# RyanXLi/OneshotDet

Hardware: AMD Instinct MI355X
Metric: images/sec/GPU fwd+bwd, 800x1024 target + 127x127 query, bs=8; 1->8 GPU scaling (higher is better)
Workload: dtype bf16; 1 GPU; BASELINE.json configs[2]: bs=8/GPU, 800x1024 target + 127x127 query, bf16 MFMA convs, forward (two R-50-FPN backbones, query pooling, correlation, FCOS head, training proposals) + FCOS loss + backward (stem/layer1 frozen) + gradient all-reduce + SGD(momentum) + weight repack; global_batch=8, parallelism=dp1: one rank, no collective anywhere in the step, world_size=1

## Files before the change

oneshotdet_amd/csrc/conv_wgrad.hip:

```cpp
#include "wgrad_params.h"

namespace {

__device__ __attribute__((aligned(256))) unsigned g_wzero[64];

__device__ __forceinline__ void wg_dma16(const void* gsrc, unsigned lds_dst) {
  unsigned keep;
  asm volatile(
      "s_mov_b32 %0, m0\n\ts_mov_b32 m0, %2\n\ts_nop 0\n\tglobal_load_lds_dwordx4 %1, off\n\ts_mov_b32 m0, %0"
      : "=&s"(keep)
      : "v"(gsrc), "s"(lds_dst)
      : "memory");
}

template <typename T, int BKP, int NST, int WCO, int WCI, int WM, int WN, bool ILV = false>
__global__ void __launch_bounds__(64 * WM * WN, (WM * WN == 4 && WCO + WCI == 3) ? 2 : 1) conv_wgrad_kernel(WgradParams gp) {
  constexpr int NW = WM * WN;
  constexpr int EPC = 16 / (int)sizeof(T);
  constexpr int TWS = 256 / (int)sizeof(T);
  constexpr int TCO = WCO * TWS, TCI = WCI * TWS;
  constexpr int OPB = BKP * 256;
  constexpr int STAGE = (WCO + WCI) * OPB;
  constexpr int PPS = BKP / 4;
  constexpr int IPA = WCO * PPS / NW;
// ... 747 lines not shown
__global__ void pred_wgrad_reduce_kernel(const float* __restrict__ part, const float* __restrict__ part_b, float* __restrict__ dw,
                                         float* __restrict__ db, int blocks, int groups, int C, int cout) {
  const int i = blockIdx.x * blockDim.x + threadIdx.x;
  const int n = cout * 9 * C;
  const int per = (blocks + gridDim.y - 1) / gridDim.y;
  const int b0 = blockIdx.y * per, b1 = min(blocks, b0 + per);
  if (i < n) {
    const int c = i % C, ct = i / C;
    const int cg = c >> 8, cl = c & 255;
    const size_t stride = (size_t)groups * 36 * 256;
    const float* p = part + ((size_t)cg * 36 + ct) * 256 + cl;
    float s0 = 0.f, s1 = 0.f, s2 = 0.f, s3 = 0.f;
    int b = b0;
    for (; b + 3 < b1; b += 4) {
      s0 += p[(size_t)b * stride]; s1 += p[(size_t)(b + 1) * stride]; s2 += p[(size_t)(b + 2) * stride]; s3 += p[(size_t)(b + 3) * stride];
    }
    for (; b < b1; ++b) s0 += p[(size_t)b * stride];
    if (b0 < b1) atomicAdd(dw + i, (s0 + s1) + (s2 + s3));
  } else if (db != nullptr && i < n + cout) {
    const int co = i - n;
    float s = 0.f;
    for (int b = b0 * 4; b < b1 * 4; ++b) s += part_b[(size_t)b * 4 + co];
    if (b0 < b1) atomicAdd(db + co, s);
  }
}

template <typename T>
__global__ void __launch_bounds__(256) bias_grad_kernel(const T* __restrict__ dy, float* __restrict__ db, int M, int C,
                                                        int stride, int rows_per_block) {
  const int c = blockIdx.y * blockDim.x + threadIdx.x;
  const int p_lo = blockIdx.x * rows_per_block, p_hi = min(M, p_lo + rows_per_block);
  if (c >= C || p_lo >= p_hi) return;
  float s = 0.f;
  for (int m = p_lo; m < p_hi; ++m) s += to_f32(dy[(size_t)m * stride + c]);
  atomicAdd(db + c, s);
}

}

#define OSD_STREAM(s) reinterpret_cast<hipStream_t>(s)

extern "C" int osd_bias_grad(const void* dy, float* db, int m, int c, int stride, int dtype, void* stream);

static bool wgrad_dense_input(const osd_conv_desc* d) {
  return d->in_stride_w == d->cin && d->in_stride_h == d->w * d->cin && (long long)d->in_stride_n == (long long)d->h * d->w * d->cin;
}

struct WgradProblem {
  const osd_conv_desc* d;
  int n, h, w;
  const void* x; const void* dy; const float* scale; float* dw; float* db;
};

static int wgrad_xr_launch(int n_seg, const WgradProblem* pr, hipStream_t s) {
  if (n_seg < 1 || n_seg > kMaxSeg) return osd_fail(OSD_ERR_INVALID_ARG, "wgrad: 1..%d segments", kMaxSeg);
  const osd_conv_desc* d0 = pr[0].d;
  static const int kTargets[8] = {512, 256, 128, 64, 1024, 768, 1536, 2048};
  const int a = d0->algo - 1 - 128;
  const int x = a & 15, target = kTargets[(a >> 4) & 7];
  if (a < 0 || a >= 128 || x > 2) return osd_fail(OSD_ERR_INVALID_ARG, "wgrad: unknown algo %d", d0->algo);
  const int bkp = x == 1 ? 64 : 32;
  WgradParams p;
  p.n_seg = n_seg;
  p.sk_units = 0;
  long long work = 0;
  for (int i = 0; i < n_seg; ++i) {
    const osd_conv_desc* d = pr[i].d;
    WgradSeg& g = p.seg[i];
    g.owner = 0;
    const int h = pr[i].h, w = pr[i].w;
    if (d->dtype != OSD_BF16 || d->r != 3 || d->s != 3 || d->stride_h != 1 || d->stride_w != 1 || d->pad_h != 1 || d->pad_w != 1 ||
        d->cout % 128 || d->cin % 128 || d->out_stride % 8 || !(w % bkp == 0 || bkp % w == 0))
      return osd_fail(OSD_ERR_UNSUPPORTED, "wgrad (filter-row kernel): bf16 3x3 / 1 / 1, channels in 128s, width %d vs %d-pixel stages", w, bkp);
    const long long M = (long long)pr[i].n * h * w;
    if (M <= 0 || M > 0x7fffffffLL || !pr[i].x || !pr[i].dy || !pr[i].dw) return osd_fail(OSD_ERR_INVALID_ARG, "wgrad: bad segment %d", i);
    if (M * d->cin > 0x7fffffffLL) return osd_fail(OSD_ERR_UNSUPPORTED, "wgrad: input of segment %d has more than 2^31 elements", i);
    g.x = pr[i].x; g.dy = pr[i].dy; g.dw = pr[i].dw; g.scale = pr[i].scale; g.db = pr[i].db;
    g.H = h; g.W = w; g.Ho = h; g.Wo = w; g.M = (int)M;
    g.Cin = d->cin; g.Cout = d->cout; g.R = 3; g.S = 3; g.sh = g.sw = 1; g.ph = g.pw = 1;
    g.dy_stride = d->out_stride; g.Ktot = 9 * d->cin;
    g.tilesCo = d->cout / 128; g.tilesCi = d->cin / 128;
    work += M * g.tilesCo * g.tilesCi * 3;
  }
  long long rows = (work + target - 1) / target;
  rows = (rows + 63) / 64 * 64;
  if (rows < 128) rows = 128;
  long long nblocks = 0;
  for (int i = 0; i < n_seg; ++i) {
    WgradSeg& g = p.seg[i];
    int sp = (int)((g.M + rows - 1) / rows);
    if (sp < 1) sp = 1;
    g.rows_per_split = cdiv(cdiv(g.M, sp), 64) * 64;
    const int splits = cdiv(g.M, g.rows_per_split);
    g.block_begin = (int)nblocks;
    nblocks += (long long)g.tilesCo * g.tilesCi * 3 * splits;
    if (nblocks > 0x7fffffffLL) return osd_fail(OSD_ERR_INVALID_ARG, "wgrad: bad grid");
  }
  for (int i = n_seg; i < kMaxSeg; ++i) p.seg[i] = p.seg[0];
  p.n_blocks = (int)nblocks;
  p.partials = nullptr;
#define OSD_WGX(BK, NS)                                                                                               \
  do {                                                                                                                \
    auto kern = conv_wgrad_xr_kernel<BK, NS>;                                                                         \
    constexpr int lds = NS * (BK + BK + 4) * 256;                                                                     \
    static bool attr = false;                                                                                         \
    if (!attr) { (void)hipFuncSetAttribute(reinterpret_cast<const void*>(kern), hipFuncAttributeMaxDynamicSharedMemorySize, lds); attr = true; } \
    hipLaunchKernelGGL(kern, dim3((unsigned)nblocks), dim3(512), lds, s, p);                                         \
  } while (0)
  if (x == 0) OSD_WGX(32, 6);
  else if (x == 1) OSD_WGX(64, 4);
  else OSD_WGX(32, 8);
#undef OSD_WGX
  return osd_check_launch("conv_wgrad_xr");
}

static int wgrad_launch_v(int n_seg, const WgradProblem* pr, hipStream_t s, int variant_override);
static int wgrad_launch(int n_seg, const WgradProblem* pr, hipStream_t s) {
  int rc = wgrad_launch_v(n_seg, pr, s, -1);
  if (rc == OSD_ERR_UNSUPPORTED && n_seg >= 1 && pr[0].d->algo == 0) rc = wgrad_launch_v(n_seg, pr, s, 0);
  return rc;
}

static int wgrad_launch_v(int n_seg, const WgradProblem* pr, hipStream_t s, int variant_override) {
  if (n_seg < 1 || n_seg > kMaxSeg) return osd_fail(OSD_ERR_INVALID_ARG, "wgrad: 1..%d segments", kMaxSeg);
  const osd_conv_desc* d0 = pr[0].d;
  if (d0->algo > 128) return wgrad_xr_launch(n_seg, pr, s);
  static int env_target = -1, env_variant = -1;
  if (env_target < 0) { const char* e = getenv("OSD_WGRAD_BLOCKS"); env_target = e ? atoi(e) : 512; }
  if (env_variant < 0) { const char* e = getenv("OSD_WGRAD_VARIANT"); env_variant = e ? atoi(e) : 0; }
  static const int kTargets[8] = {512, 256, 128, 64, 1024, 768, 1536, 2048};
  int target = env_target, variant = variant_override >= 0 ? variant_override : env_variant, code = 0;
  if (d0->algo > 0) {
    const int a = d0->algo - 1;
    if (a >= 128) return osd_fail(OSD_ERR_INVALID_ARG, "wgrad: unknown algo %d", d0->algo);
    variant = a & 15;
    code = a >> 4;
    target = kTargets[code];
  }
  if (d0->dtype == OSD_F32) target *= 8;
  const bool bf = d0->dtype == OSD_BF16;
  if (!bf && variant != 0) variant = 0;
  const int sub_co = bf && (variant == 3 || variant == 4 || variant == 5 || variant == 7 || variant == 8 || variant == 9 || variant == 11 || variant == 13 || variant == 14) ? 2 : 1;
  const int sub_ci = bf && (variant == 3 || variant == 4 || variant == 5 || variant == 6 || variant == 8 || variant == 9 || variant == 10 || variant == 13) ? 2 : 1;
  const int tw = bf ? 128 : 64;
  const int epc = d0->dtype == OSD_BF16 ? 8 : 4;
  WgradParams p;
  p.n_seg = n_seg;
  long long work = 0;
  for (int i = 0; i < n_seg; ++i) {
    const osd_conv_desc* d = pr[i].d;
    WgradSeg& g = p.seg[i];
    if (d->dtype != d0->dtype) return osd_fail(OSD_ERR_INVALID_ARG, "wgrad: segments of different dtype");
    if (d->cin % epc || d->out_stride % epc) return osd_fail(OSD_ERR_INVALID_ARG, "wgrad: channel counts must keep 16-byte alignment");
    const int ho = (pr[i].h + 2 * d->pad_h - d->r) / d->stride_h + 1, wo = (pr[i].w + 2 * d->pad_w - d->s) / d->stride_w + 1;
    const long long M = (long long)pr[i].n * ho * wo;
    if (M <= 0 || M > 0x7fffffffLL || !pr[i].x || !pr[i].dy || !pr[i].dw) return osd_fail(OSD_ERR_INVALID_ARG, "wgrad: bad segment %d", i);
    if ((long long)pr[i].n * pr[i].h * pr[i].w * d->cin > 0x7fffffffLL)
      return osd_fail(OSD_ERR_UNSUPPORTED, "wgrad: input of segment %d has more than 2^31 elements", i);
    g.x = pr[i].x; g.dy = pr[i].dy; g.dw = pr[i].dw; g.scale = pr[i].scale; g.db = pr[i].db;
    g.H = pr[i].h; g.W = pr[i].w; g.Ho = ho; g.Wo = wo; g.M = (int)M;
    g.Cin = d->cin; g.Cout = d->cout; g.R = d->r; g.S = d->s;
    g.sh = d->stride_h; g.sw = d->stride_w; g.ph = d->pad_h; g.pw = d->pad_w;
    g.dy_stride = d->out_stride; g.Ktot = d->r * d->s * d->cin;
    g.tilesCo = cdiv(d->cout, tw * sub_co); g.tilesCi = cdiv(d->cin, tw * sub_ci);
    work += M * g.tilesCo * g.tilesCi * d->r * d->s;
  }
  long long rows = (work + target - 1) / target;
  rows = (rows + 31) / 32 * 32;
  if (rows < 128) rows = 128;
  long long nblocks = 0;
  for (int i = 0; i < n_seg; ++i) {
    WgradSeg& g = p.seg[i];
    int sp = (int)((g.M + rows - 1) / rows);
    if (sp < 1) sp = 1;
    g.rows_per_split = cdiv(cdiv(g.M, sp), 32) * 32;
    const int splits = cdiv(g.M, g.rows_per_split);
    g.owner = splits == 1 ? 1 : 0;
    g.block_begin = (int)nblocks;
    nblocks += (long long)g.tilesCo * g.tilesCi * g.R * g.S * splits;
    if (nblocks > 0x7fffffffLL) return osd_fail(OSD_ERR_INVALID_ARG, "wgrad: bad grid");
  }
  p.sk_units = p.sk_teams = p.sk_total = 0;
  if (bf && variant == 3) {
    if (d0->ordered_ws != nullptr) return osd_fail(OSD_ERR_UNSUPPORTED, "wgrad: team mode adds its partial tiles atomically (not for ordered mode)");
    if (code > 3) return osd_fail(OSD_ERR_UNSUPPORTED, "wgrad: team mode knows target codes 0..3 (rounds)");
    const WgradSeg& g0 = p.seg[0];
    long long total = 0;
    for (int i = 0; i < n_seg; ++i) {
      WgradSeg& g = p.seg[i];
      if (g.Cout != g0.Cout || g.Cin != g0.Cin || g.R != g0.R || g.S != g0.S)
        return osd_fail(OSD_ERR_UNSUPPORTED, "wgrad: team mode needs segments of one conv shape (segment %d differs)", i);
      g.stage_begin = (int)total;
      total += cdiv(g.M, 64);
    }
    static int cus = 0;
    if (cus == 0) {
      int dev = 0;
      if (hipGetDevice(&dev) != hipSuccess || hipDeviceGetAttribute(&cus, hipDeviceAttributeMultiprocessorCount, dev) != hipSuccess || cus < 1) cus = 256;
      const char* e = getenv("OSD_WGRAD_TEAM_CUS");
      if (e && atoi(e) > 0) cus = atoi(e);
    }
    const int units = g0.tilesCo * g0.tilesCi * g0.R * g0.S;
    long long teams = (long long)cus * (code + 1) / units;
    if (teams < 1) return osd_fail(OSD_ERR_UNSUPPORTED, "wgrad: team mode needs at most one output tile x tap per CU (%d)", units);
    if (teams > total) teams = total;
    if (total > 0x7fffffffLL) return osd_fail(OSD_ERR_INVALID_ARG, "wgrad: bad grid");
    p.sk_units = units; p.sk_teams = (int)teams; p.sk_total = (int)total;
    nblocks = teams * units;
  }
  static int no_owner = -1;
  if (no_owner < 0) { const char* e = getenv("OSD_WGRAD_NO_OWNER"); no_owner = (e && atoi(e) != 0) ? 1 : 0; }
  for (int i = 0; i < n_seg; ++i) {
    if (no_owner || d0->ordered_ws != nullptr || p.sk_units > 0) p.seg[i].owner = 0;
    for (int j = 0; j < n_seg && p.seg[i].owner; ++j)
      if (j != i && p.seg[j].dw == p.seg[i].dw) p.seg[i].owner = 0;
  }
  for (int i = n_seg; i < kMaxSeg; ++i) p.seg[i] = p.seg[0];
  p.n_blocks = (int)nblocks;
  p.partials = nullptr;
  const int tco = tw * sub_co, tci = tw * sub_ci;
  if (d0->ordered_ws != nullptr) {
    const long long need = nblocks * ((long long)tco * tci + tco) * 4;
    if (need > (long long)d0->ordered_ws_bytes)
      return osd_fail(OSD_ERR_WORKSPACE, "wgrad (ordered mode): the launch needs %lld bytes of partial tiles, ordered_ws_bytes is %lld",
                      need, (long long)d0->ordered_ws_bytes);
    p.partials = static_cast<float*>(d0->ordered_ws);
  }
  const osd_conv_desc* d = d0;
#define OSD_WG_LAUNCH(TT, BK, NS, WC, WMM, WNN) OSD_WG_LAUNCH3(TT, BK, NS, WC, WC, WMM, WNN, false)
#define OSD_WG_LAUNCH2(TT, BK, NS, WCOO, WCII, WMM, WNN) OSD_WG_LAUNCH3(TT, BK, NS, WCOO, WCII, WMM, WNN, false)
#define OSD_WG_LAUNCH3(TT, BK, NS, WCOO, WCII, WMM, WNN, IL)                                                        \
  do {                                                                                                               \
    auto kern = conv_wgrad_kernel<TT, BK, NS, WCOO, WCII, WMM, WNN, IL>;                                                 \
    constexpr int lds = NS * (WCOO + WCII) * BK * 256;                                                               \
    static bool attr = false;                                                                                        \
    if (!attr) { (void)hipFuncSetAttribute(reinterpret_cast<const void*>(kern), hipFuncAttributeMaxDynamicSharedMemorySize, lds); attr = true; } \
    hipLaunchKernelGGL(kern, dim3((unsigned)nblocks), dim3(64 * WMM * WNN), lds, s, p);                             \
  } while (0)
  if (d->dtype == OSD_F32) {
    OSD_WG_LAUNCH(float, 32, 3, 1, 2, 2);
  } else {
    switch (variant) {
      case 1: OSD_WG_LAUNCH(__bf16, 64, 2, 1, 2, 2); break;
      case 2: OSD_WG_LAUNCH(__bf16, 32, 4, 1, 2, 2); break;
      case 4: OSD_WG_LAUNCH(__bf16, 32, 3, 2, 2, 4); break;
      case 5: OSD_WG_LAUNCH(__bf16, 64, 2, 2, 2, 4); break;
      case 6: OSD_WG_LAUNCH2(__bf16, 64, 2, 1, 2, 2, 4); break;
      case 7: OSD_WG_LAUNCH2(__bf16, 64, 2, 2, 1, 4, 2); break;
      case 8: OSD_WG_LAUNCH(__bf16, 32, 5, 2, 2, 4); break;
      case 9: OSD_WG_LAUNCH(__bf16, 32, 4, 2, 2, 4); break;
      case 10: OSD_WG_LAUNCH2(__bf16, 32, 3, 1, 2, 2, 2); break;
      case 11: OSD_WG_LAUNCH2(__bf16, 32, 3, 2, 1, 2, 2); break;
      case 12: return osd_fail(OSD_ERR_UNSUPPORTED, "wgrad: variant 12 is retired");
      case 3:
      case 13: {
        for (int i = 0; i < n_seg; ++i) {
          const WgradSeg& g = p.seg[i];
          if (g.Wo < 2 || g.Ho < 2 || (long long)g.M * g.Wo >= 0xffffffffLL || (long long)g.M * g.dy_stride * 2 >= 0x7fffffffLL ||
              (long long)(g.M / (g.Ho * g.Wo)) * g.H * g.W * g.Cin * 2 >= 0x7fffffffLL)
            return osd_fail(OSD_ERR_UNSUPPORTED, "wgrad: the pipelined variants need output maps of at least 2 x 2 and operands below 2 GiB (segment %d)", i);
        }
        const int rc = osd_wgrad_sk_launch(p, s);
        if (rc) return rc;
        break;
      }
      case 14: OSD_WG_LAUNCH3(__bf16, 32, 3, 2, 1, 2, 2, true); break;
      case 15: OSD_WG_LAUNCH3(__bf16, 32, 3, 1, 1, 2, 2, true); break;
      default: OSD_WG_LAUNCH(__bf16, 32, 3, 1, 2, 2); break;
    }
  }
#undef OSD_WG_LAUNCH
#undef OSD_WG_LAUNCH2
#undef OSD_WG_LAUNCH3
  if (p.partials != nullptr) {
    int rc = osd_check_launch("conv_wgrad");
    if (rc) return rc;
    long long tiles = 0;
    for (int i = 0; i < n_seg; ++i) tiles += (long long)p.seg[i].tilesCo * p.seg[i].tilesCi * p.seg[i].R * p.seg[i].S;
    hipLaunchKernelGGL(wgrad_reduce_kernel, dim3((unsigned)tiles, tco / 16), dim3(256), 0, s, p, tco, tci);
    return osd_check_launch("conv_wgrad(reduce)");
  }
  return osd_check_launch("conv_wgrad");
}

extern "C" int osd_conv2d_wgrad(const osd_conv_desc* d, const void* x, const void* dy, const float* scale, float* dw,
                                float* db, void* stream) {
  if (!d || !x || !dy || !dw) return osd_fail(OSD_ERR_INVALID_ARG, "wgrad: null argument");
  if (d->dtype != OSD_F32 && d->dtype != OSD_BF16) return osd_fail(OSD_ERR_INVALID_ARG, "wgrad: bad dtype");
  const int epc = d->dtype == OSD_BF16 ? 8 : 4;
  const long long M = (long long)d->n * d->ho * d->wo;
  if (M <= 0 || M > 0x7fffffffLL) return osd_fail(OSD_ERR_INVALID_ARG, "wgrad: bad M");
  if (!wgrad_dense_input(d)) return osd_fail(OSD_ERR_UNSUPPORTED, "wgrad: dense NHWC input required");
  hipStream_t s = OSD_STREAM(stream);
  if (d->cout <= 8 && (d->out_stride % epc != 0 || d->cin % epc != 0)) {
    if (d->r * d->s > 9) return osd_fail(OSD_ERR_UNSUPPORTED, "wgrad: skinny kernel supports up to 9 taps");
    const int rows = 512;
    dim3 grid(cdiv((int)M, rows), cdiv(d->cin, 256));
    if (d->dtype == OSD_F32)
      hipLaunchKernelGGL(conv_wgrad_skinny_kernel<float>, grid, dim3(256), 0, s, (const float*)x, (const float*)dy, dw, d->h,
                         d->w, d->cin, d->ho, d->wo, d->cout, d->r, d->s, d->stride_h, d->pad_h, d->out_stride, (int)M, rows);
    else
      hipLaunchKernelGGL(conv_wgrad_skinny_kernel<__bf16>, grid, dim3(256), 0, s, (const __bf16*)x, (const __bf16*)dy, dw,
                         d->h, d->w, d->cin, d->ho, d->wo, d->cout, d->r, d->s, d->stride_h, d->pad_h, d->out_stride, (int)M,
                         rows);
    int rc = osd_check_launch("conv_wgrad_skinny");
    if (rc || !db) return rc;
    return osd_bias_grad(dy, db, (int)M, d->cout, d->out_stride, d->dtype, stream);
  }
  const WgradProblem pr = {d, d->n, d->h, d->w, x, dy, scale, dw, db};
  return wgrad_launch(1, &pr, s);
}

extern "C" int osd_conv2d_wgrad_grouped(const osd_conv_desc* d, int n_seg, const void* const* xs, const void* const* dys,
                                        const int32_t* ns, const int32_t* hs, const int32_t* ws, const float* scale,
// ... 216 lines not shown
  const unsigned blocks = (unsigned)cdiv(cin * kPredG, 256);
  if (dtype == OSD_F32)
    hipLaunchKernelGGL(pred_dgrad_pack_kernel<float>, dim3(blocks), dim3(256), 0, OSD_STREAM(stream), w, (float*)wd, cout, cin);
  else
    hipLaunchKernelGGL(pred_dgrad_pack_kernel<__bf16>, dim3(blocks), dim3(256), 0, OSD_STREAM(stream), w, (__bf16*)wd, cout, cin);
  return osd_check_launch("pred_dgrad_pack");
}

extern "C" int osd_conv2d_wgrad_pred_gathered(const osd_conv_desc* d, int n_seg, const void* const* xs, const void* g, const int32_t* ns,
                                              const int32_t* hs, const int32_t* ws, float* dw, float* db, void* workspace, void* stream) {
  if (!xs || !g || !dw || !workspace) return osd_fail(OSD_ERR_INVALID_ARG, "wgrad_pred_gathered: null argument");
  int rc = pred_check("wgrad_pred_gathered", d, n_seg, ns, hs, ws);
  if (rc) return rc;
  for (int i = 0; i < n_seg; ++i)
    if (!xs[i]) return osd_fail(OSD_ERR_INVALID_ARG, "wgrad_pred_gathered: null segment %d", i);
  return pred_wgrad_from_g(d, n_seg, xs, g, ns, hs, ws, dw, db, workspace, OSD_STREAM(stream));
}

extern "C" int osd_conv2d_wgrad_batched(const osd_conv_desc* d, int n_seg, const void* const* xs, const void* const* dys,
                                        const float* const* scales, float* const* dws, float* const* dbs, void* stream) {
  if (!d || !xs || !dys || !dws || n_seg < 1 || n_seg > kMaxSeg)
    return osd_fail(OSD_ERR_INVALID_ARG, "wgrad_batched: bad arguments");
  if (d->dtype != OSD_F32 && d->dtype != OSD_BF16) return osd_fail(OSD_ERR_INVALID_ARG, "wgrad: bad dtype");
  if (!wgrad_dense_input(d)) return osd_fail(OSD_ERR_UNSUPPORTED, "wgrad_batched: dense NHWC input required");
  WgradProblem pr[kMaxSeg];
  for (int i = 0; i < n_seg; ++i)
    pr[i] = WgradProblem{d, d->n, d->h, d->w, xs[i], dys[i], scales ? scales[i] : nullptr, dws[i], dbs ? dbs[i] : nullptr};
  return wgrad_launch(n_seg, pr, OSD_STREAM(stream));
}

extern "C" int osd_conv2d_wgrad_multi(const osd_conv_desc* d, int n_seg, const void* const* xs, const void* const* dys,
                                      const int32_t* ns, const int32_t* hs, const int32_t* ws, const float* const* scales,
                                      float* const* dws, float* const* dbs, void* stream) {
  if (!d || !xs || !dys || !ns || !hs || !ws || !dws || n_seg < 1 || n_seg > kMaxSeg)
    return osd_fail(OSD_ERR_INVALID_ARG, "wgrad_multi: bad arguments (1..%d segments)", kMaxSeg);
  if (d->dtype != OSD_F32 && d->dtype != OSD_BF16) return osd_fail(OSD_ERR_INVALID_ARG, "wgrad: bad dtype");
  WgradProblem pr[kMaxSeg];
  for (int i = 0; i < n_seg; ++i)
    pr[i] = WgradProblem{d, ns[i], hs[i], ws[i], xs[i], dys[i], scales ? scales[i] : nullptr, dws[i], dbs ? dbs[i] : nullptr};
  return wgrad_launch(n_seg, pr, OSD_STREAM(stream));
}

extern "C" int osd_conv2d_wgrad_mixed(int n_seg, const osd_conv_desc* descs, const void* const* xs, const void* const* dys,
                                      const float* const* scales, float* const* dws, float* const* dbs, void* stream) {
  if (!descs || !xs || !dys || !dws || n_seg < 1 || n_seg > kMaxSeg)
    return osd_fail(OSD_ERR_INVALID_ARG, "wgrad_mixed: bad arguments (1..%d segments)", kMaxSeg);
  if (descs[0].dtype != OSD_F32 && descs[0].dtype != OSD_BF16) return osd_fail(OSD_ERR_INVALID_ARG, "wgrad: bad dtype");
  WgradProblem pr[kMaxSeg];
  for (int i = 0; i < n_seg; ++i) {
    const osd_conv_desc* d = descs + i;
    if (!wgrad_dense_input(d)) return osd_fail(OSD_ERR_UNSUPPORTED, "wgrad_mixed: dense NHWC input required (segment %d)", i);
    pr[i] = WgradProblem{d, d->n, d->h, d->w, xs[i], dys[i], scales ? scales[i] : nullptr, dws[i], dbs ? dbs[i] : nullptr};
  }
  return wgrad_launch(n_seg, pr, OSD_STREAM(stream));
}

extern "C" int osd_bias_grad(const void* dy, float* db, int m, int c, int stride, int dtype, void* stream) {
  if (!dy || !db) return osd_fail(OSD_ERR_INVALID_ARG, "bias_grad: null argument");
  if (m == 0 || c == 0) return OSD_OK;
  const int rows = m > 65536 ? 2048 : 512;
  dim3 grid(cdiv(m, rows), cdiv(c, 256));
  if (dtype == OSD_F32)
    hipLaunchKernelGGL(bias_grad_kernel<float>, grid, dim3(256), 0, OSD_STREAM(stream), (const float*)dy, db, m, c, stride, rows);
  else if (dtype == OSD_BF16)
    hipLaunchKernelGGL(bias_grad_kernel<__bf16>, grid, dim3(256), 0, OSD_STREAM(stream), (const __bf16*)dy, db, m, c, stride,
                       rows);
  else
    return osd_fail(OSD_ERR_INVALID_ARG, "bias_grad: bad dtype");
  return osd_check_launch("bias_grad");
}
```

oneshotdet_amd/ops.py:

```python
import ctypes as C
import os

import torch

from . import _lib, spec
from ._lib import (ACT_EXP_SCALE, ACT_NONE, ACT_RELU, GN_SPLITS, OSD_BF16, OSD_F32, RES_DOWN2X, RES_NONE, RES_SAME, RES_UP2X,
                   ConvDesc)

__all__ = ["ACT_NONE", "ACT_RELU", "ACT_EXP_SCALE", "RES_NONE", "RES_SAME", "RES_UP2X", "RES_DOWN2X"]


from . import streams

_stream_handle = streams.raw_handle


def _stream():
    return C.c_void_p(_stream_handle())


from .trace import rec as _rec
from . import trace as _trace


# ... 51 lines not shown
        scale = (g * var.rsqrt()).contiguous()
        fbias = b - mean * scale
    else:
        fbias = bias.float() if bias is not None else torch.zeros(cout, device=weight.device)
    cout_store = _round_up(cout, 4)
    w_rows = _round_up(cout, 16)
    bias_p = torch.zeros(_round_up(cout_store, 16), device=weight.device, dtype=torch.float32)
    bias_p[:cout] = fbias
    if stem:
        assert (cin, r, s) == (3, 7, 7)
        wp = torch.empty((w_rows, 7, 32), device=weight.device, dtype=dtype)
        _lib.call("osd_pack_stem_weight", _p(weight), _p(scale), _p(wp), cout, w_rows, _dt(wp), _stream())
        return PackedConv(wp, bias_p, cout, cout_store, w_rows, 32, 7, 1, stem=True, cin_real=3)
    mult = 64 if dtype == torch.bfloat16 else 16
    cin_pad = _round_up(cin, mult)
    wp = torch.empty((w_rows, r, s, cin_pad), device=weight.device, dtype=dtype)
    _lib.call("osd_pack_conv_weight", _p(weight), _p(scale), _p(wp), cout, cin, r, s, w_rows, cin_pad, _dt(wp),
              _stream())
    return PackedConv(wp, bias_p, cout, cout_store, w_rows, cin_pad, r, s, cin_real=cin)


def pack_image(images, dtype, hp, wp, pad_t=3, pad_l=3):
    _chk_dev(images)
    n, c, h, w = images.shape
    assert c == 3 and images.dtype == torch.float32
    out = torch.empty((n, hp, wp, 4), device=images.device, dtype=dtype)
    _lib.call("osd_pack_image", _ptr(images.contiguous()), _p(out), n, h, w, hp, wp, pad_t, pad_l, _dt(out), _stream())
    _rec("pack_image", x=images, out=out, pad_t=pad_t, pad_l=pad_l)
    return out


class PackedImages(object):

    def __init__(self, tensor, hw, image_sizes):
        self.tensor, self.hw, self.image_sizes = tensor, tuple(hw), [tuple(s) for s in image_sizes]

    @property
    def shape(self):
        return (self.tensor.shape[0], 3, self.hw[0], self.hw[1])


def stem_input(images, dtype):
    n, _, h, w = images.shape
    ho, wo = conv_out(h, 7, 2, 3), conv_out(w, 7, 2, 3)
    if isinstance(images, PackedImages):
        assert images.tensor.dtype == dtype, "PackedImages were written as %s, the engine computes in %s" % (images.tensor.dtype, dtype)
        return images.tensor, (ho, wo)
    hp, wp = max(2 * (ho - 1) + 7, h + 3), max(2 * (wo - 1) + 8, w + 3)
    wp += wp & 1
    return pack_image(images, dtype, hp, wp), (ho, wo)


from .tuner import (TUNE_LOG, refine_in_step, wgrad_timer, ALGO_CACHE, CONV_ALGO_PX, CONV_ALGO_PX_WIDE, SPLIT_CACHE, WGRAD_ALGO_CACHE, _TUNING, _candidate_runs, _photo_finish, _time_launches, _tune, _tune_wgrad,
                    conv_algo_candidates, replaying, tuning, wgrad_algo_candidates, wgrad_xr_candidates)


class ConvSrc2(C.Structure):
    _fields_ = [("x", C.c_void_p), ("w2", C.c_void_p), ("cin2", C.c_int32), ("h", C.c_int32), ("w", C.c_int32),
                ("stride", C.c_int32)]


def conv2d(x, pc, stride=1, pad=0, act=ACT_NONE, res=None, res_mode=RES_NONE, relu_in=False, act_scale=1.0, out=None,
           out_hw=None, algo=None, mask=None, act_scale_dev=None, x2=None, x2_stride=1, pc2=None, bias=None):
    _chk_dev(x, res, out)
    if x2 is not None:
        return _conv2d_two_sources(x, x2, x2_stride, pc, act, out, algo, pc2, bias)
    shape = x.shape
    okey = None if out is None else out.shape[-1]
    ckey = (shape, x.dtype, pc.cout_store, pc.w_rows, pc.cin_k, pc.r, pc.s, pc.stem, stride, pad, act, res_mode,
            None if res is None else res.shape, bool(relu_in), float(act_scale), mask is not None, out_hw, okey)
    ent = _CONV_DESCS.get(ckey)
    if ent is None:
        ent = _CONV_DESCS[ckey] = _build_conv_desc(x, pc, stride, pad, act, res, res_mode, relu_in, act_scale, out, out_hw, mask)
    d, oshape, key = ent[0], ent[1], ent[2]
    if out is None:
        out = torch.empty(oshape, device=x.device, dtype=x.dtype)
    if mask is not None:
        assert mask.shape == out.shape and mask.dtype == out.dtype
    args = (_p(x), _p(pc.w), _p(pc.bias), _p(res), _p(mask), _p(act_scale_dev), None, _p(out), _stream())
    if algo is None:
        algo = ALGO_CACHE.get(key)
        if algo is None:
            algo = _tune(key, d, lambda: _lib.call("osd_conv2d_fwd", C.byref(d), *args), prewarm=lambda: x.float().sum()) if _TUNING[0] else 0
    d.algo = algo
    try:
        _lib.call("osd_conv2d_fwd", C.byref(d), *args)
    except _lib.OsdError as e:
        if getattr(e, "code", 0) != -2 or algo == 0 or ALGO_CACHE.get(key) != algo:
            raise
        del ALGO_CACHE[key]
        d.algo = 0
        _lib.call("osd_conv2d_fwd", C.byref(d), *args)
    _rec("conv", x=x, w=pc.w, bias=pc.bias, cout=pc.cout_store, r=pc.r, s=pc.s, stem=pc.stem, stride=stride, pad=pad, act=act,
         res=res, res_mode=res_mode, relu_in=bool(relu_in), act_scale=float(act_scale), act_scale_dev=act_scale_dev, mask=mask,
         out=out, algo=d.algo, key=key)
    return out


_CONV_DESCS = {}


def _p(t):
    return None if t is None else t.data_ptr()


def _build_conv_desc(x, pc, stride, pad, act, res, res_mode, relu_in, act_scale, out, out_hw, mask):
    n, h, w, c = x.shape
# ... 758 lines not shown
        dbp = (C.c_void_p * k)(*[(t.data_ptr() if t is not None else 0) for t in dbs])
        _lib.call("osd_conv2d_wgrad_batched", C.byref(d), k, xs, dys, scales, dwp, dbp, st)
    key = ("batched", k, d.dtype, tuple(x0.shape), cout, r, s, stride, pad, dy0.shape[-1], has_db, _wgrad_mode())
    if algo is None:
        algo = WGRAD_ALGO_CACHE.get(key)
    if algo is None:
        if _TUNING[0]:
            sdw = [torch.empty_like(it[2]) for it in items]
            sdb = [None if it[4] is None else torch.empty_like(it[4]) for it in items]
            algo = _tune_wgrad(key, d, lambda a, b: launch(sdw, sdb), items[0][2], None, [x0.shape[2]])
        else:
            algo = 0
    d.algo = algo
    launch([it[2] for it in items], [it[4] for it in items])
    _rec("wgrad", items=[dict(x=it[0], dy=it[1], dw=it[2], scale=it[3], db=it[4], r=r, s=s, stride=stride, pad=pad, cout=cout)
                         for it in items], algo=algo, key=key)


def conv2d_wgrad_multi(items, r, s, stride, pad, cout, algo=None):
    x0, dy0 = items[0][0], items[0][1]
    d = _conv_desc(x0.shape, _dt(x0), cout, r, s, stride, pad, dy0.shape[-1])
    k = len(items)
    xs = (C.c_void_p * k)(*[it[0].data_ptr() for it in items])
    dys = (C.c_void_p * k)(*[it[1].data_ptr() for it in items])
    ns = (C.c_int32 * k)(*[it[0].shape[0] for it in items])
    hs = (C.c_int32 * k)(*[it[0].shape[1] for it in items])
    ws = (C.c_int32 * k)(*[it[0].shape[2] for it in items])
    scales = (C.c_void_p * k)(*[(it[3].data_ptr() if it[3] is not None else 0) for it in items])
    st = _stream()
    real_dws, real_dbs = [it[2] for it in items], [it[4] for it in items]

    def launch(dws, dbs):
        dwp = (C.c_void_p * k)(*[t.data_ptr() for t in dws])
        dbp = (C.c_void_p * k)(*[(t.data_ptr() if t is not None else 0) for t in dbs])
        _lib.call("osd_conv2d_wgrad_multi", C.byref(d), k, xs, dys, ns, hs, ws, scales, dwp, dbp, st)
    key = ("multi", d.dtype, tuple(tuple(it[0].shape) for it in items), tuple(id(it[2]) == id(items[0][2]) for it in items),
           cout, r, s, stride, pad, dy0.shape[-1], any(b is not None for b in real_dbs), _wgrad_mode())
    if algo is None:
        algo = WGRAD_ALGO_CACHE.get(key)
    if algo is None:
        if _TUNING[0]:
            scratch = {}
            sdw = [scratch.setdefault(id(t), torch.empty_like(t)) for t in real_dws]
            sdb = [None if t is None else scratch.setdefault(id(t), torch.empty_like(t)) for t in real_dbs]
            algo = _tune_wgrad(key, d, lambda a, b: launch(sdw, sdb), real_dws[0], None, [it[0].shape[2] for it in items])
        else:
            algo = 0
    d.algo = algo
    launch(real_dws, real_dbs)
    _rec("wgrad", items=[dict(x=it[0], dy=it[1], dw=it[2], scale=it[3], db=it[4], r=r, s=s, stride=stride, pad=pad, cout=cout)
                         for it in items], algo=algo, key=key)


def conv2d_wgrad_mixed(items, algo=None):
    k = len(items)
    descs = (ConvDesc * k)()
    for i, (x, dy, dw, scale, db, r, s, stride, pad, cout) in enumerate(items):
        d = _conv_desc(x.shape, _dt(x), cout, r, s, stride, pad, dy.shape[-1])
        assert (dy.shape[1], dy.shape[2]) == (d.ho, d.wo), (x.shape, dy.shape)
        descs[i] = d
    xs = (C.c_void_p * k)(*[it[0].data_ptr() for it in items])
    dys = (C.c_void_p * k)(*[it[1].data_ptr() for it in items])
    scales = (C.c_void_p * k)(*[(it[3].data_ptr() if it[3] is not None else 0) for it in items])
    st = _stream()
    real_dws, real_dbs = [it[2] for it in items], [it[4] for it in items]

    def launch(dws, dbs):
        dwp = (C.c_void_p * k)(*[t.data_ptr() for t in dws])
        dbp = (C.c_void_p * k)(*[(t.data_ptr() if t is not None else 0) for t in dbs])
        _lib.call("osd_conv2d_wgrad_mixed", k, descs, xs, dys, scales, dwp, dbp, st)
    key = ("mixed", descs[0].dtype, tuple((tuple(it[0].shape), tuple(it[1].shape)) + tuple(it[5:]) for it in items),
           tuple([id(u) for u in real_dws].index(id(t)) for t in real_dws), _wgrad_mode())
    if algo is None:
        algo = WGRAD_ALGO_CACHE.get(key)
    if algo is None:
        if _TUNING[0]:
            scratch = {}
            sdw = [scratch.setdefault(id(t), torch.empty_like(t)) for t in real_dws]
            sdb = [None if t is None else scratch.setdefault(id(t), torch.empty_like(t)) for t in real_dbs]
            timed = []
            timer = wgrad_timer()
            for cand in wgrad_algo_candidates(descs[0].dtype, max(d.cout for d in descs), max(d.cin for d in descs)):
                descs[0].algo = cand
                if not _candidate_runs(lambda: launch(sdw, sdb)):
                    continue
                timed.append((timer(lambda: launch(sdw, sdb)), cand))

            def retime(cand):
                descs[0].algo = cand
                return timer(lambda: launch(sdw, sdb))
            WGRAD_ALGO_CACHE[key] = algo = _photo_finish(timed, retime)
            TUNE_LOG["WGRAD_ALGO_CACHE"][key] = sorted(timed)
        else:
            algo = 0
    descs[0].algo = algo
    launch(real_dws, real_dbs)
    _rec("wgrad", items=[dict(x=it[0], dy=it[1], dw=it[2], scale=it[3], db=it[4], r=it[5], s=it[6], stride=it[7], pad=it[8],
                              cout=it[9]) for it in items], algo=algo, key=key)


def bias_grad(dy, db, c):
    n, h, w, stride = dy.shape
    _lib.call("osd_bias_grad", _p(dy), _p(db), n * h * w, c, stride, _dt(dy), _stream())


def unpack_wgrad(dw_packed, scale=None, out=None, accumulate=False):
    _chk_dev(dw_packed, scale, out)
    cout, r, s, cin = dw_packed.shape
    if out is None:
        if accumulate:
            raise ValueError("unpack_wgrad: accumulate needs the tensor to add to")
        out = torch.empty((cout, cin, r, s), device=dw_packed.device, dtype=torch.float32)
    _lib.call("osd_unpack_wgrad", _p(dw_packed), _p(scale), _p(out), cout, cin, r, s, int(bool(accumulate)), _stream())
    return out


def conv2d_dgrad_naive(dy, w_fwd_packed, x_shape, r, s, stride, pad, cout, mask=None, addend=None):
    d = _conv_desc(x_shape, _dt(dy), cout, r, s, stride, pad, dy.shape[-1])
    dx = torch.empty(x_shape, device=dy.device, dtype=dy.dtype)
    _lib.call("osd_conv2d_dgrad_naive", C.byref(d), _p(dy), _p(w_fwd_packed), _p(mask), _p(addend), _p(dx),
              _stream())
    return dx


def scatter2x(src, out_hw, mask=None, addend=None):
    n, ho, wo, c = src.shape
    h, w = out_hw
    dst = torch.empty((n, h, w, c), device=src.device, dtype=src.dtype)
    _lib.call("osd_scatter2x", _p(src), _p(mask), _p(addend), _p(dst), n, h, w, ho, wo, c, _dt(src), _stream())
    _rec("scatter2x", x=src, mask=mask, addend=addend, out=dst)
    return dst


def add_mask(a, b=None, mask=None, out=None):
    out = torch.empty_like(a) if out is None else out
    _lib.call("osd_add_mask", _p(a), _p(b), _p(mask), _p(out), a.numel(), _dt(a), _stream())
    _rec("add_mask", a=a, b=b, mask=mask, out=out)
    return out


def upsample2x_bwd(inner, prev=None):
    n, h2, w2, c = inner.shape
    if h2 % 2 or w2 % 2:
        raise ValueError("upsample2x_bwd: the gradient map must have even height and width, got %d x %d" % (h2, w2))
    top = torch.empty((n, h2 // 2, w2 // 2, c), device=inner.device, dtype=inner.dtype)
    _lib.call("osd_upsample2x_bwd", _p(inner), _p(prev), _p(top), n, h2 // 2, w2 // 2, c, _dt(inner), _stream())
    _rec("upsample2x_bwd", inner=inner, prev=prev, out=top)
    return top


def correlate_bwd_query(g, feat):
# ... 422 lines not shown
```

oneshotdet_amd/tuner.py:

```python
import os

import torch

from . import _lib
from ._lib import OSD_BF16

class _Cache(dict):
    census = False

    def __init__(self, *a, **kw):
        dict.__init__(self, *a, **kw)
        self.hits = {}

    def get(self, key, default=None):
        if self.census:
            self.hits[key] = self.hits.get(key, 0) + 1
        return dict.get(self, key, default)


SPLIT_CACHE = _Cache()
WGRAD_ALGO_CACHE = _Cache()
TUNE_LOG = {"ALGO_CACHE": {}, "WGRAD_ALGO_CACHE": {}, "SPLIT_CACHE": {}}

ALGO_CACHE = _Cache()
# ... 124 lines not shown

def _tune(key, d, launch, cands=None, prewarm=None):
    timed = []
    pixels = d.n * d.ho * d.wo
    cold = 0 < pixels <= COLD_MAX_PIXELS and d.cout > 16 and not os.environ.get("OSD_TUNE_WARM_ONLY")
    time_it = (lambda f: _time_launches_cold(f, prewarm)) if cold else _time_launches
    forced = os.environ.get("OSD_FORCE_ALGO_3X3_256")
    if forced and d.cout == 256 and d.r == 3 and d.stride_h == 1:
        d.algo = int(forced)
        try:
            launch()
            torch.cuda.synchronize()
            ALGO_CACHE[key] = int(forced)
            return int(forced)
        except _lib.OsdError:
            pass
    for algo in (cands if cands is not None else conv_algo_candidates(d.cout, d.relu_in, has_mask=bool(key[-1]), pixels=pixels if pixels > 0 else None)):
        d.algo = algo
        try:
            launch()
        except _lib.OsdError:
            continue
        timed.append((time_it(launch), algo))

    def retime(algo):
        d.algo = algo
        return time_it(launch)
    best = _photo_finish(timed, retime)
    ALGO_CACHE[key] = best
    TUNE_LOG["ALGO_CACHE"][key] = sorted(timed)
    return best


def wgrad_xr_candidates(dtype, cout, cin, r, s, stride, pad, widths):
    if dtype != OSD_BF16 or (r, s, stride, pad) != (3, 3, 1, 1) or cout % 128 or cin % 128 or not widths:
        return []
    xs = [x for x, bk in ((0, 32), (1, 64), (2, 32)) if all(w % bk == 0 or bk % w == 0 for w in widths)]
    return [1 + 128 + x + 16 * t for t in (0, 1, 2, 4, 5, 6, 7) for x in xs]


def wgrad_algo_candidates(dtype, cout=0, cin=0):
    variants = [0, 1, 2] if dtype == OSD_BF16 else [0]
    if dtype == OSD_BF16:
        variants.append(15)
    if dtype == OSD_BF16 and cout >= 256 and cin >= 256:
        variants += [3, 4, 5, 8, 9, 13]
    if dtype == OSD_BF16 and cin >= 256:
        variants += [6, 10]
    if dtype == OSD_BF16 and cout >= 256:
        variants += [7, 11, 14]
    excl = [int(v) for v in os.environ.get("OSD_WGRAD_EXCLUDE", "").split(",") if v]
    variants = [v for v in variants if v not in excl]
    return [1 + v + 16 * t for t in (0, 1, 2, 3, 4, 5, 6, 7) for v in variants if not (v == 3 and t > 3)]


def _candidate_runs(fn):
    try:
        fn()
        return True
    except _lib.OsdError as e:
        if getattr(e, "code", 0) == -2:
            return False
        raise


def wgrad_timer():
    return _time_launches_cold if os.environ.get("OSD_TUNE_WGRAD_COLD") else _time_launches


def _tune_wgrad(key, d, launch, dw, db, widths=None):
    _time_launches = wgrad_timer()
    sdw = torch.empty_like(dw)
    sdb = None if db is None else torch.empty_like(db)
    timed = []
    cands = wgrad_algo_candidates(d.dtype, d.cout, d.cin)
    if os.environ.get("OSD_WGRAD_XR"):
        cands = cands + wgrad_xr_candidates(d.dtype, d.cout, d.cin, d.r, d.s, d.stride_h, d.pad_h, widths)
    verbose = os.environ.get("OSD_TUNE_VERBOSE")
    for algo in cands:
        d.algo = algo
        if not _candidate_runs(lambda: launch(sdw, sdb)):
            if verbose:
                print("   wgrad tuner: variant %d code %d refused" % ((algo - 1) & 15, (algo - 1) >> 4))
            continue
        t = _time_launches(lambda: launch(sdw, sdb))
        if verbose:
            print("   wgrad tuner: variant %d code %d  %.1f us" % ((algo - 1) & 15, (algo - 1) >> 4, t * 1e3))
        timed.append((t, algo))

    def retime(algo):
        d.algo = algo
        return _time_launches(lambda: launch(sdw, sdb))
    best = _photo_finish(timed, retime)
    WGRAD_ALGO_CACHE[key] = best
    TUNE_LOG["WGRAD_ALGO_CACHE"][key] = sorted(timed)
    return best


def refine_in_step(step, sync, n_steps=12, margin=0.10, min_share=0.004, gain=0.003, budget_s=100.0, verbose=False, cycle=1):
    import time
    caches = {"ALGO_CACHE": ALGO_CACHE, "WGRAD_ALGO_CACHE": WGRAD_ALGO_CACHE, "SPLIT_CACHE": SPLIT_CACHE}

    n_steps = (n_steps + cycle - 1) // cycle * cycle

    def measure():
        evs = []
# ... 60 lines not shown
```

Baseline: 769.0 images/sec.

## Split grouped wgrad launch into per-class algos tuned separately

Partitions the segments of a mixed weight-gradient call into classes: wide 3x3 stride-1 convs keyed by channel count, narrow convs, and the rest. Each class is tuned for its own kernel algo, and the C launcher issues one launch per class after a dry-run validation pass over all classes. The split is kept only if it beats the single whole-group algo by a margin. The aim is to stop heterogeneous segments being forced onto one tile configuration, at the cost of extra launches and a longer tuning time.

```diff
diff --git a/oneshotdet_amd/csrc/conv_wgrad.hip b/oneshotdet_amd/csrc/conv_wgrad.hip
--- a/oneshotdet_amd/csrc/conv_wgrad.hip
+++ b/oneshotdet_amd/csrc/conv_wgrad.hip
@@ -823,7 +823,7 @@
   const void* x; const void* dy; const float* scale; float* dw; float* db;
 };
 
-static int wgrad_xr_launch(int n_seg, const WgradProblem* pr, hipStream_t s) {
+static int wgrad_xr_launch(int n_seg, const WgradProblem* pr, hipStream_t s, bool dry) {
   if (n_seg < 1 || n_seg > kMaxSeg) return osd_fail(OSD_ERR_INVALID_ARG, "wgrad: 1..%d segments", kMaxSeg);
   const osd_conv_desc* d0 = pr[0].d;
   static const int kTargets[8] = {512, 256, 128, 64, 1024, 768, 1536, 2048};
@@ -870,6 +870,7 @@
   for (int i = n_seg; i < kMaxSeg; ++i) p.seg[i] = p.seg[0];
   p.n_blocks = (int)nblocks;
   p.partials = nullptr;
+  if (dry) return OSD_OK;
 #define OSD_WGX(BK, NS)                                                                                               \
   do {                                                                                                                \
     auto kern = conv_wgrad_xr_kernel<BK, NS>;                                                                         \
@@ -885,17 +886,17 @@
   return osd_check_launch("conv_wgrad_xr");
 }
 
-static int wgrad_launch_v(int n_seg, const WgradProblem* pr, hipStream_t s, int variant_override);
-static int wgrad_launch(int n_seg, const WgradProblem* pr, hipStream_t s) {
-  int rc = wgrad_launch_v(n_seg, pr, s, -1);
-  if (rc == OSD_ERR_UNSUPPORTED && n_seg >= 1 && pr[0].d->algo == 0) rc = wgrad_launch_v(n_seg, pr, s, 0);
+static int wgrad_launch_v(int n_seg, const WgradProblem* pr, hipStream_t s, int variant_override, bool dry);
+static int wgrad_launch(int n_seg, const WgradProblem* pr, hipStream_t s, bool dry = false) {
+  int rc = wgrad_launch_v(n_seg, pr, s, -1, dry);
+  if (rc == OSD_ERR_UNSUPPORTED && n_seg >= 1 && pr[0].d->algo == 0) rc = wgrad_launch_v(n_seg, pr, s, 0, dry);
   return rc;
 }
 
-static int wgrad_launch_v(int n_seg, const WgradProblem* pr, hipStream_t s, int variant_override) {
+static int wgrad_launch_v(int n_seg, const WgradProblem* pr, hipStream_t s, int variant_override, bool dry) {
   if (n_seg < 1 || n_seg > kMaxSeg) return osd_fail(OSD_ERR_INVALID_ARG, "wgrad: 1..%d segments", kMaxSeg);
   const osd_conv_desc* d0 = pr[0].d;
-  if (d0->algo > 128) return wgrad_xr_launch(n_seg, pr, s);
+  if (d0->algo > 128) return wgrad_xr_launch(n_seg, pr, s, dry);
   static int env_target = -1, env_variant = -1;
   if (env_target < 0) { const char* e = getenv("OSD_WGRAD_BLOCKS"); env_target = e ? atoi(e) : 512; }
   if (env_variant < 0) { const char* e = getenv("OSD_WGRAD_VARIANT"); env_variant = e ? atoi(e) : 0; }
@@ -997,6 +998,16 @@
                       need, (long long)d0->ordered_ws_bytes);
     p.partials = static_cast<float*>(d0->ordered_ws);
   }
+  if (bf && variant == 12) return osd_fail(OSD_ERR_UNSUPPORTED, "wgrad: variant 12 is retired");
+  if (bf && (variant == 3 || variant == 13)) {
+    for (int i = 0; i < n_seg; ++i) {
+      const WgradSeg& g = p.seg[i];
+      if (g.Wo < 2 || g.Ho < 2 || (long long)g.M * g.Wo >= 0xffffffffLL || (long long)g.M * g.dy_stride * 2 >= 0x7fffffffLL ||
+          (long long)(g.M / (g.Ho * g.Wo)) * g.H * g.W * g.Cin * 2 >= 0x7fffffffLL)
+        return osd_fail(OSD_ERR_UNSUPPORTED, "wgrad: the pipelined variants need output maps of at least 2 x 2 and operands below 2 GiB (segment %d)", i);
+    }
+  }
+  if (dry) return OSD_OK;
   const osd_conv_desc* d = d0;
 #define OSD_WG_LAUNCH(TT, BK, NS, WC, WMM, WNN) OSD_WG_LAUNCH3(TT, BK, NS, WC, WC, WMM, WNN, false)
 #define OSD_WG_LAUNCH2(TT, BK, NS, WCOO, WCII, WMM, WNN) OSD_WG_LAUNCH3(TT, BK, NS, WCOO, WCII, WMM, WNN, false)
@@ -1022,15 +1033,8 @@
       case 9: OSD_WG_LAUNCH(__bf16, 32, 4, 2, 2, 4); break;
       case 10: OSD_WG_LAUNCH2(__bf16, 32, 3, 1, 2, 2, 2); break;
       case 11: OSD_WG_LAUNCH2(__bf16, 32, 3, 2, 1, 2, 2); break;
-      case 12: return osd_fail(OSD_ERR_UNSUPPORTED, "wgrad: variant 12 is retired");
       case 3:
       case 13: {
-        for (int i = 0; i < n_seg; ++i) {
-          const WgradSeg& g = p.seg[i];
-          if (g.Wo < 2 || g.Ho < 2 || (long long)g.M * g.Wo >= 0xffffffffLL || (long long)g.M * g.dy_stride * 2 >= 0x7fffffffLL ||
-              (long long)(g.M / (g.Ho * g.Wo)) * g.H * g.W * g.Cin * 2 >= 0x7fffffffLL)
-            return osd_fail(OSD_ERR_UNSUPPORTED, "wgrad: the pipelined variants need output maps of at least 2 x 2 and operands below 2 GiB (segment %d)", i);
-        }
         const int rc = osd_wgrad_sk_launch(p, s);
         if (rc) return rc;
         break;
@@ -1353,7 +1357,40 @@
     if (!wgrad_dense_input(d)) return osd_fail(OSD_ERR_UNSUPPORTED, "wgrad_mixed: dense NHWC input required (segment %d)", i);
     pr[i] = WgradProblem{d, d->n, d->h, d->w, xs[i], dys[i], scales ? scales[i] : nullptr, dws[i], dbs ? dbs[i] : nullptr};
   }
-  return wgrad_launch(n_seg, pr, OSD_STREAM(stream));
+  int cls[kMaxSeg], n_cls = 0, cls_algo[kMaxSeg];
+  for (int i = 0; i < n_seg; ++i) {
+    const int a = (i == 0 || descs[i].algo == 0) ? descs[0].algo : descs[i].algo;
+    int c = 0;
+    while (c < n_cls && cls_algo[c] != a) ++c;
+    if (c == n_cls) cls_algo[n_cls++] = a;
+    cls[i] = c;
+  }
+  if (n_cls == 1) return wgrad_launch(n_seg, pr, OSD_STREAM(stream));
+  WgradProblem sub[kMaxSeg];
+  osd_conv_desc head[kMaxSeg];
+  int begin[kMaxSeg + 1];
+  begin[0] = 0;
+  for (int c = 0; c < n_cls; ++c) {
+    int k = begin[c];
+    for (int i = 0; i < n_seg; ++i) {
+      if (cls[i] != c) continue;
+      if (descs[i].dtype != descs[0].dtype) return osd_fail(OSD_ERR_INVALID_ARG, "wgrad: segments of different dtype");
+      sub[k++] = pr[i];
+    }
+    head[c] = *sub[begin[c]].d;
+    head[c].algo = cls_algo[c];
+    head[c].ordered_ws = descs[0].ordered_ws;
+    head[c].ordered_ws_bytes = descs[0].ordered_ws_bytes;
+    sub[begin[c]].d = &head[c];
+    begin[c + 1] = k;
+  }
+  for (int pass = 0; pass < 2; ++pass) {
+    for (int c = 0; c < n_cls; ++c) {
+      const int rc = wgrad_launch(begin[c + 1] - begin[c], sub + begin[c], OSD_STREAM(stream), pass == 0);
+      if (rc) return rc;
+    }
+  }
+  return OSD_OK;
 }
 
 extern "C" int osd_bias_grad(const void* dy, float* db, int m, int c, int stride, int dtype, void* stream) {
diff --git a/oneshotdet_amd/ops.py b/oneshotdet_amd/ops.py
--- a/oneshotdet_amd/ops.py
+++ b/oneshotdet_amd/ops.py
@@ -127,7 +127,7 @@
 
 
 from .tuner import (TUNE_LOG, refine_in_step, wgrad_timer, ALGO_CACHE, CONV_ALGO_PX, CONV_ALGO_PX_WIDE, SPLIT_CACHE, WGRAD_ALGO_CACHE, _TUNING, _candidate_runs, _photo_finish, _time_launches, _tune, _tune_wgrad,
-                    conv_algo_candidates, replaying, tuning, wgrad_algo_candidates, wgrad_xr_candidates)
+                    conv_algo_candidates, replaying, tuning, wgrad_algo_candidates, wgrad_class_partition, wgrad_xr_candidates)
 
 
 class ConvSrc2(C.Structure):
@@ -992,7 +992,7 @@
                          for it in items], algo=algo, key=key)
 
 
-def conv2d_wgrad_mixed(items, algo=None):
+def _wgrad_mixed_call(items):
     k = len(items)
     descs = (ConvDesc * k)()
     for i, (x, dy, dw, scale, db, r, s, stride, pad, cout) in enumerate(items):
@@ -1003,40 +1003,105 @@
     dys = (C.c_void_p * k)(*[it[1].data_ptr() for it in items])
     scales = (C.c_void_p * k)(*[(it[3].data_ptr() if it[3] is not None else 0) for it in items])
     st = _stream()
-    real_dws, real_dbs = [it[2] for it in items], [it[4] for it in items]
 
     def launch(dws, dbs):
         dwp = (C.c_void_p * k)(*[t.data_ptr() for t in dws])
         dbp = (C.c_void_p * k)(*[(t.data_ptr() if t is not None else 0) for t in dbs])
         _lib.call("osd_conv2d_wgrad_mixed", k, descs, xs, dys, scales, dwp, dbp, st)
-    key = ("mixed", descs[0].dtype, tuple((tuple(it[0].shape), tuple(it[1].shape)) + tuple(it[5:]) for it in items),
-           tuple([id(u) for u in real_dws].index(id(t)) for t in real_dws), _wgrad_mode())
-    if algo is None:
-        algo = WGRAD_ALGO_CACHE.get(key)
-    if algo is None:
-        if _TUNING[0]:
-            scratch = {}
-            sdw = [scratch.setdefault(id(t), torch.empty_like(t)) for t in real_dws]
-            sdb = [None if t is None else scratch.setdefault(id(t), torch.empty_like(t)) for t in real_dbs]
-            timed = []
-            timer = wgrad_timer()
-            for cand in wgrad_algo_candidates(descs[0].dtype, max(d.cout for d in descs), max(d.cin for d in descs)):
-                descs[0].algo = cand
-                if not _candidate_runs(lambda: launch(sdw, sdb)):
-                    continue
-                timed.append((timer(lambda: launch(sdw, sdb)), cand))
-
-            def retime(cand):
-                descs[0].algo = cand
-                return timer(lambda: launch(sdw, sdb))
-            WGRAD_ALGO_CACHE[key] = algo = _photo_finish(timed, retime)
-            TUNE_LOG["WGRAD_ALGO_CACHE"][key] = sorted(timed)
-        else:
-            algo = 0
-    descs[0].algo = algo
-    launch(real_dws, real_dbs)
-    _rec("wgrad", items=[dict(x=it[0], dy=it[1], dw=it[2], scale=it[3], db=it[4], r=it[5], s=it[6], stride=it[7], pad=it[8],
-                              cout=it[9]) for it in items], algo=algo, key=key)
+    return descs, launch
+
+
+def _wgrad_mixed_key(items):
+    dws = [id(it[2]) for it in items]
+    return ("mixed", _dt(items[0][0]), tuple((tuple(it[0].shape), tuple(it[1].shape)) + tuple(it[5:]) for it in items),
+            tuple(dws.index(t) for t in dws), _wgrad_mode())
+
+
+def _tune_wgrad_mixed(items, key):
+    descs, launch = _wgrad_mixed_call(items)
+    scratch = {}
+    sdw = [scratch.setdefault(id(it[2]), torch.empty_like(it[2])) for it in items]
+    sdb = [None if it[4] is None else scratch.setdefault(id(it[4]), torch.empty_like(it[4])) for it in items]
+    timed = []
+    timer = wgrad_timer()
+    for cand in wgrad_algo_candidates(descs[0].dtype, max(d.cout for d in descs), max(d.cin for d in descs)):
+        descs[0].algo = cand
+        if not _candidate_runs(lambda: launch(sdw, sdb)):
+            continue
+        timed.append((timer(lambda: launch(sdw, sdb)), cand))
+
+    def retime(cand):
+        descs[0].algo = cand
+        return timer(lambda: launch(sdw, sdb))
+    WGRAD_ALGO_CACHE[key] = algo = _photo_finish(timed, retime)
+    TUNE_LOG["WGRAD_ALGO_CACHE"][key] = sorted(timed)
+    return algo
+
+
+WGRAD_CLASSES_MARGIN = 0.05
+
+
+def _wgrad_classes_win(items, classes, whole_algo):
+    descs, launch = _wgrad_mixed_call(items)
+    scratch = {}
+    sdw = [scratch.setdefault(id(it[2]), torch.empty_like(it[2])) for it in items]
+    sdb = [None if it[4] is None else scratch.setdefault(id(it[4]), torch.empty_like(it[4])) for it in items]
+    timer = wgrad_timer()
+    best = [float("inf"), float("inf")]
+    for _ in range(3):
+        for which in (0, 1):
+            for idx, a, _ in classes:
+                for i in idx:
+                    descs[i].algo = a if which == 0 else whole_algo
+            best[which] = min(best[which], timer(lambda: launch(sdw, sdb)))
+    TUNE_LOG["WGRAD_ALGO_CACHE"][("classes-vs-one",) + _wgrad_mixed_key(items)[1:]] = [(best[0], "classes"), (best[1], "one")]
+    return best[0] < best[1] * (1.0 - WGRAD_CLASSES_MARGIN)
+
+
+def conv2d_wgrad_mixed(items, algo=None):
+    k = len(items)
+    everything = list(range(k))
+    if isinstance(algo, (list, tuple)):
+        assert len(algo) == k, (len(algo), k)
+        ids = [int(algo[0])] + [int(a) or int(algo[0]) for a in algo[1:]]
+        classes = [([i for i in everything if ids[i] == a], a) for a in dict.fromkeys(ids)]
+        classes = [(idx, a, _wgrad_mixed_key([items[i] for i in idx])) for idx, a in classes]
+    elif algo is not None:
+        classes = [(everything, algo, _wgrad_mixed_key(items))]
+    else:
+        classes = []
+        x0 = items[0][0]
+        parts = wgrad_class_partition(_dt(x0), [(x.shape[-1], cout, r, s, stride, pad, dy.shape[0], dy.shape[1], dy.shape[2])
+                                                for x, dy, _, _, _, r, s, stride, pad, cout in items])
+        whole = _wgrad_mixed_key(items)
+        if len(parts) > 1 and whole not in WGRAD_ALGO_CACHE:
+            subs = [[items[i] for i in idx] for idx in parts]
+            keys = [_wgrad_mixed_key(sub) for sub in subs]
+            if _TUNING[0] or all(key in WGRAD_ALGO_CACHE for key in keys):
+                ids = [WGRAD_ALGO_CACHE.get(key) for key in keys]
+                fresh = [key for key, a in zip(keys, ids) if a is None]
+                ids = [_tune_wgrad_mixed(sub, key) if a is None else a for sub, key, a in zip(subs, keys, ids)]
+                if all(ids):
+                    classes = list(zip(parts, ids, keys))
+                if fresh and not (classes and _wgrad_classes_win(items, classes, _tune_wgrad_mixed(items, whole))):
+                    for key in keys:
+                        WGRAD_ALGO_CACHE.pop(key, None)
+                    classes = []
+                elif fresh:
+                    WGRAD_ALGO_CACHE.pop(whole, None)
+        if not classes:
+            a = WGRAD_ALGO_CACHE.get(whole)
+            if a is None:
+                a = _tune_wgrad_mixed(items, whole) if _TUNING[0] else 0
+            classes = [(everything, a, whole)]
+    descs, launch = _wgrad_mixed_call(items)
+    for idx, a, _ in classes:
+        for i in idx:
+            descs[i].algo = a
+    launch([it[2] for it in items], [it[4] for it in items])
+    for idx, a, key in classes:
+        _rec("wgrad", items=[dict(x=it[0], dy=it[1], dw=it[2], scale=it[3], db=it[4], r=it[5], s=it[6], stride=it[7], pad=it[8],
+                                  cout=it[9]) for it in (items[i] for i in idx)], algo=a, key=key)
 
 
 def bias_grad(dy, db, c):
diff --git a/oneshotdet_amd/tuner.py b/oneshotdet_amd/tuner.py
--- a/oneshotdet_amd/tuner.py
+++ b/oneshotdet_amd/tuner.py
@@ -200,6 +200,41 @@
     excl = [int(v) for v in os.environ.get("OSD_WGRAD_EXCLUDE", "").split(",") if v]
     variants = [v for v in variants if v not in excl]
     return [1 + v + 16 * t for t in (0, 1, 2, 3, 4, 5, 6, 7) for v in variants if not (v == 3 and t > 3)]
+
+
+WGRAD_CLASS_MIN_SHARE = 0.05
+
+
+def wgrad_class_partition(dtype, shapes, min_share=WGRAD_CLASS_MIN_SHARE):
+    everything = [list(range(len(shapes)))]
+    if dtype != OSD_BF16 or len(shapes) < 2 or os.environ.get("OSD_WGRAD_CLASSES", "1") == "0":
+        return everything
+    labels, flop = [], {}
+    for cin, cout, r, s, stride, pad, n, ho, wo in shapes:
+        if (r, s, stride, pad) == (3, 3, 1, 1) and min(cin, cout) >= 256 and min(ho, wo) >= 2:
+            lab = ("team", cin, cout)
+        elif min(cin, cout) <= 128:
+            lab = ("narrow",)
+        else:
+            lab = ("rest",)
+        labels.append(lab)
+        flop[lab] = flop.get(lab, 0.0) + 2.0 * n * ho * wo * cout * cin * r * s
+    total = sum(flop.values())
+    if total <= 0:
+        return everything
+    small = [lab for lab in flop if lab != ("rest",) and flop[lab] < min_share * total]
+    for lab in small:
+        flop[("rest",)] = flop.get(("rest",), 0.0) + flop.pop(lab)
+    labels = [("rest",) if lab in small else lab for lab in labels]
+    if ("rest",) in flop and flop[("rest",)] < min_share * total and len(flop) > 1:
+        flop.pop(("rest",))
+        biggest = max(flop, key=flop.get)
+        labels = [biggest if lab == ("rest",) else lab for lab in labels]
+    order = []
+    for lab in labels:
+        if lab not in order:
+            order.append(lab)
+    return [[i for i, lab in enumerate(labels) if lab == o] for o in order]
 
 
 def _candidate_runs(fn):
```

Result: no change. 768.7 images/sec, median of 2 (-0.0%).
